# Ecogenomics/CheckM

Measured on NVIDIA H100. Metric: genomes/hour, higher is better.
Workload: dtype int16 (SSV) / u8 (MSV) / int16 (Viterbi) / f32 (Forward, domain definition)

## Files before the change

checkm_b200/csrc/kernels_vitp.cu:

```cuda
#include "engine.hpp"
#include "device_utils.cuh"
#include "stages.hpp"

namespace ckm {

constexpr uint32_t VP_FLOORW = 0xD800D800u;
constexpr int      VP_FLOOR  = -10240;
constexpr uint32_t VP_TFLOORW = 0xC000C000u;

__device__ __forceinline__ int vp_lo(uint32_t w) { return (int)(int16_t)(w & 0xffffu); }
__device__ __forceinline__ int vp_hi(uint32_t w) { return (int)w >> 16; }

__device__ __forceinline__ void vit_pass(const FilterParams &p, const Candidate &cd) {
  const int pos = atomicAdd(p.out_count, 1);
  if (pos < p.out_cap) p.out[pos] = cd;
  if (p.dense_passed != nullptr) atomicOr_u8(p.dense_passed, (int64_t)p.model_slot[cd.model] * p.nseq + cd.seq, 4);
}
__device__ __forceinline__ void vit_redo(const FilterParams &p, const Candidate &cd) {
  const int pos = atomicAdd(p.redo_count, 1);
  if (pos < p.redo_cap) p.redo[pos] = cd;
}
__device__ __forceinline__ int vitp_class(int vq) { return vq == 0 ? -1 : (vq <= 8 ? vq / 2 - 1 : vq / 4 + 1); }

__global__ void vit_count_kernel(FilterParams p, int32_t *cnt) {
  const int n = min(*p.in_count, p.in_cap);
  for (int i = blockIdx.x * blockDim.x + threadIdx.x; i < n; i += gridDim.x * blockDim.x) {
    const Candidate cd = p.in[i];
    if (!(cd.P > p.F2)) vit_pass(p, cd);
    else if (p.ms[cd.model].vq == 0) vit_redo(p, cd);
    else atomicAdd(cnt + cd.model, 1);
  }
}

__global__ void __launch_bounds__(1024) vit_scan_kernel(FilterParams p, int32_t nmodels, const int32_t *cnt, int32_t *off, int32_t *choff) {
  __shared__ int ws[2][32];
  const int lane = threadIdx.x & 31, warp = threadIdx.x >> 5;
  int run_pairs = 0, run_chunks = 0;
  for (int c = 0; c < N_BLK_CLASSES; ++c) {
    if (threadIdx.x == 0) p.vit_cls_chunks[c] = run_chunks;
    for (int b = 0; b < nmodels; b += 1024) {
      const int m = b + threadIdx.x;
      const int v = (m < nmodels && vitp_class(p.ms[m].vq) == c) ? cnt[m] : 0, h = (v + VITP_CHUNK - 1) / VITP_CHUNK;
      int sv = v, sh = h;
#pragma unroll
      for (int o = 1; o < 32; o <<= 1) {
        const int a = __shfl_up_sync(0xffffffffu, sv, o), d = __shfl_up_sync(0xffffffffu, sh, o);
        if (lane >= o) { sv += a; sh += d; }
      }
      if (lane == 31) { ws[0][warp] = sv; ws[1][warp] = sh; }
      __syncthreads();
      if (warp == 0) {
        int tv = ws[0][lane], th = ws[1][lane];
#pragma unroll
        for (int o = 1; o < 32; o <<= 1) {
          const int a = __shfl_up_sync(0xffffffffu, tv, o), d = __shfl_up_sync(0xffffffffu, th, o);
          if (lane >= o) { tv += a; th += d; }
        }
        ws[0][lane] = tv; ws[1][lane] = th;
      }
      __syncthreads();
      if (v > 0) {
        off[m] = run_pairs + (warp ? ws[0][warp - 1] : 0) + sv - v;
        choff[m] = run_chunks + (warp ? ws[1][warp - 1] : 0) + sh - h;
      }
      run_pairs += ws[0][31]; run_chunks += ws[1][31];
      __syncthreads();
    }
  }
  if (threadIdx.x == 0) p.vit_cls_chunks[N_BLK_CLASSES] = run_chunks;
}

__global__ void vit_scatter_kernel(FilterParams p, const int32_t *cnt, int32_t *fill, const int32_t *off, const int32_t *choff) {
  const int n = min(*p.in_count, p.in_cap);
  for (int i = blockIdx.x * blockDim.x + threadIdx.x; i < n; i += gridDim.x * blockDim.x) {
    const int m = p.in[i].model;
    if (!(p.in[i].P > p.F2) || p.ms[m].vq == 0) continue;
    const int r = atomicAdd(fill + m, 1), pos = off[m] + r;
    p.vit_idx[pos] = i;
    if (r % VITP_CHUNK == 0) p.vit_chunks[choff[m] + r / VITP_CHUNK] = make_int2(pos, off[m] + min(r + VITP_CHUNK, cnt[m]));
  }
}

int launch_vit_group(const FilterParams &p, int32_t nmodels, int32_t *ws, int grid, cudaStream_t st) {
  int32_t *cnt = ws, *fill = ws + nmodels, *off = ws + 2 * (size_t)nmodels, *choff = ws + 3 * (size_t)nmodels;
  cudaError_t e = cudaMemsetAsync(ws, 0, sizeof(int32_t) * 2 * (size_t)nmodels, st);
  if (e != cudaSuccess) return cuda_fail(e, "cudaMemsetAsync(vit groups)");
  vit_count_kernel<<<grid, 256, 0, st>>>(p, cnt);
  vit_scan_kernel<<<1, 1024, 0, st>>>(p, nmodels, cnt, off, choff);
  vit_scatter_kernel<<<grid, 256, 0, st>>>(p, cnt, fill, off, choff);
  e = cudaGetLastError();
  return e == cudaSuccess ? CKM_OK : cuda_fail(e, "vit grouping launch");
}

constexpr int VITP_THREADS = 128;

__host__ __device__ constexpr int vitp_smem_bytes(int W, bool tsmem) { return KPAD * W * 32 * 4 + (tsmem ? W * 64 * 16 : 0); }
__host__ __device__ constexpr int vitp_min_blocks(int W) { return W <= 4 ? 4 : (W <= 10 ? 3 : 2); }

template <int W, bool TSMEM>
__global__ void __launch_bounds__(VITP_THREADS, vitp_min_blocks(W)) vitp_kernel(FilterParams p, int cls) {
  extern __shared__ __align__(16) uint4 vsm[];
  __shared__ int s_chunk, s_next;
  __shared__ ModelScalars s_ms;
  uint32_t *esm = reinterpret_cast<uint32_t *>(vsm);
  uint4 *tws = vsm + KPAD * W * 8;
  const int lane = threadIdx.x & 31;
  const uint32_t sel = (lane == 0) ? 0x1054u : 0x3210u;
  const int c0 = p.vit_cls_chunks[cls], nch = p.vit_cls_chunks[cls + 1] - c0;
  for (;;) {
    __syncthreads();
    if (threadIdx.x == 0) {
      const int k = atomicAdd(p.vit_work + cls, 1);
      s_chunk = k;
      if (k < nch) {
        s_next = p.vit_chunks[c0 + k].x;
        s_ms = p.ms[p.in[p.vit_idx[s_next]].model];
      }
    }
    __syncthreads();
    const int k = s_chunk;
    if (k >= nch) break;
    const int2 ch = p.vit_chunks[c0 + k];
    const ModelScalars &ms = s_ms;
    {
      const uint4 *esrc = reinterpret_cast<const uint4 *>(p.rwp + ms.blk_off * 32 * (KPAD / 2));
      for (int z = threadIdx.x; z < KPAD * W * 8; z += VITP_THREADS) vsm[z] = __ldg(esrc + z);
      if (TSMEM) {
        const uint4 *tsrc = p.twp + ms.blk_off * 32;
        for (int z = threadIdx.x; z < W * 64; z += VITP_THREADS) tws[(z & 1) * (W * 32) + (z >> 1)] = __ldg(tsrc + z);
      }
    }
    uint4 tr0[TSMEM ? 1 : W], tr1[TSMEM ? 1 : W];
    if (!TSMEM) {
      const uint4 *tsrc = p.twp + ms.blk_off * 32;
#pragma unroll
      for (int w = 0; w < W; ++w) { tr0[TSMEM ? 0 : w] = __ldg(tsrc + (w * 32 + lane) * 2); tr1[TSMEM ? 0 : w] = __ldg(tsrc + (w * 32 + lane) * 2 + 1); }
    }
#define TR0(w) (TSMEM ? tws[(w) * 32 + lane] : tr0[TSMEM ? 0 : (w)])
#define TR1(w) (TSMEM ? tws[W * 32 + (w) * 32 + lane] : tr1[TSMEM ? 0 : (w)])
    __syncthreads();
    const uint32_t *erow = esm + lane;
    const int ddbound = ms.ddbound_w, cap = 32767 - (int)ms.vit_emax;
    const int e_move = ms.xw_e_move, e_loop = ms.xw_e_loop;
    for (;;) {
      int j = 0;
      if (lane == 0) j = atomicAdd(&s_next, 1);
      j = __shfl_sync(0xffffffffu, j, 0);
      if (j >= ch.y) break;
      const Candidate *cin = p.in + p.vit_idx[j];
      const int s = cin->seq, L = p.len[s];
      bool redo = false;
      const int tmove = p.tmove_w[s];
      const int cost = -tmove - (int)ms.vit_tbm + 64;
      const bool c1 = (cost - (int)ms.xw_e_loop <= 22528) && (cost <= 22240);
      const bool c1p = (cost - (int)ms.xw_e_loop <= 16384);
      redo = !c1;
      float vsc = 0.0f;
      if (!redo) {
        uint32_t Mx[W], Ix[W], Dx[W];
#pragma unroll
        for (int w = 0; w < W; ++w) { Mx[w] = VP_FLOORW; Ix[w] = VP_FLOORW; Dx[w] = VP_FLOORW; }
        int xN = ms.base_w, xB = xN + tmove, xJ = -32768, xC = -32768;
        const uint32_t *rp = reinterpret_cast<const uint32_t *>(p.res + p.off[s]);
        const int nw = (L + 3) >> 2;
        uint32_t wcur = (nw > 0) ? __ldg(rp) : 0u;
        bool stop = false;
        for (int q = 0; q < nw && !stop; ++q) {
          const uint32_t wnext = (q + 1 < nw) ? __ldg(rp + q + 1) : 0u;
#pragma unroll
          for (int rr = 0; rr < 4; ++rr) {
            if (q * 4 + rr >= L) { stop = true; break; }
            const uint32_t *ew = erow + ((wcur >> (8 * rr)) & 0xffu) * (W * 32);
            const uint32_t shM = __shfl_sync(0xffffffffu, Mx[W - 1], (lane + 31) & 31);
            const uint32_t shI = __shfl_sync(0xffffffffu, Ix[W - 1], (lane + 31) & 31);
            const uint32_t shD = __shfl_sync(0xffffffffu, Dx[W - 1], (lane + 31) & 31);
            const uint32_t pm0 = __byte_perm(shM, VP_FLOORW, sel), pi0 = __byte_perm(shI, VP_FLOORW, sel), pd0 = __byte_perm(shD, VP_FLOORW, sel);
            const uint32_t xBw = __byte_perm((uint32_t)xB, 0u, 0x1010u);
            uint32_t md[W];
            uint32_t xEw = VP_FLOORW, dmw = VP_FLOORW;
#pragma unroll
            for (int w = W - 1; w >= 0; --w) {
              const uint32_t pm = (w > 0) ? Mx[w - 1] : pm0, pi = (w > 0) ? Ix[w - 1] : pi0, pd = (w > 0) ? Dx[w - 1] : pd0;
              const uint4 t0 = TR0(w), t1 = TR1(w);
              uint32_t sv = __viaddmax_s16x2(xBw, t0.x, VP_FLOORW);
              sv = __viaddmax_s16x2(pm, t0.y, sv);
              sv = __viaddmax_s16x2(pi, t0.z, sv);
              sv = __viaddmax_s16x2(pd, t0.w, sv);
              sv = __viaddmax_s16x2(sv, ew[w * 32], VP_FLOORW);
              const uint32_t nI = __viaddmax_s16x2(Ix[w], t1.z, __viaddmax_s16x2(Mx[w], t1.y, VP_FLOORW));
              md[w] = __viaddmax_s16x2(sv, t1.x, VP_FLOORW);
              Mx[w] = sv; Ix[w] = nI;
            }
#pragma unroll
            for (int w = 0; w + 1 < W; w += 2) { xEw = __vimax3_s16x2(xEw, Mx[w], Mx[w + 1]); dmw = __vimax3_s16x2(dmw, md[w], md[w + 1]); }
            if (W & 1) { xEw = __vimax3_s16x2(xEw, Mx[W - 1], Mx[W - 1]); dmw = __vimax3_s16x2(dmw, md[W - 1], md[W - 1]); }
            const int xE = __reduce_max_sync(0xffffffffu, max(vp_lo(xEw), vp_hi(xEw)));
            if (xE >= cap) { redo = true; stop = true; break; }
            xC = max(xC, xE + e_move);
            xJ = max(xJ, xE + e_loop);
            xB = max(xJ + tmove, xN + tmove);
            const int Dmax = __reduce_max_sync(0xffffffffu, max(vp_lo(dmw), vp_hi(dmw)));
            if (Dmax + ddbound > xB) {
              if (!c1p) { redo = true; stop = true; break; }
              uint32_t Bb = VP_FLOORW, Tb = 0u;
#pragma unroll
              for (int w = 0; w < W; ++w) { const uint32_t tdd = TR1(w).w; Bb = __viaddmax_s16x2(Bb, tdd, md[w]); Tb = __viaddmax_s16x2(Tb, __vimax3_s16x2(tdd, VP_TFLOORW, VP_TFLOORW), VP_TFLOORW); }
              uint32_t Bs = Bb, Ts = Tb;
#pragma unroll
              for (int o = 1; o < 32; o <<= 1) {
                const uint32_t Bl = __shfl_up_sync(0xffffffffu, Bs, o), Tl = __shfl_up_sync(0xffffffffu, Ts, o);
                if (lane >= o) { Bs = __viaddmax_s16x2(Bl, Ts, Bs); Ts = __viaddmax_s16x2(Ts, Tl, VP_TFLOORW); }
              }
              uint32_t din = __shfl_up_sync(0xffffffffu, Bs, 1), Tex = __shfl_up_sync(0xffffffffu, Ts, 1);
              if (lane == 0) { din = VP_FLOORW; Tex = 0u; }
              const uint32_t lowexit = __shfl_sync(0xffffffffu, Bs, 31);
              const uint32_t dmid = __byte_perm(lowexit, VP_FLOORW, 0x1054u);
              din = __viaddmax_s16x2(dmid, Tex, din);
              uint32_t d = din;
#pragma unroll
              for (int w = 0; w < W; ++w) { Dx[w] = d; d = __viaddmax_s16x2(d, TR1(w).w, md[w]); }
            } else {
              const uint32_t shd = __shfl_sync(0xffffffffu, md[W - 1], (lane + 31) & 31);
#pragma unroll
              for (int w = W - 1; w >= 1; --w) Dx[w] = md[w - 1];
              Dx[0] = __byte_perm(shd, VP_FLOORW, sel);
            }
          }
          wcur = wnext;
        }
        if (!redo && xC <= VP_FLOOR + e_move) redo = true;
        if (!redo) {
          vsc = __fsub_rn(__fadd_rn((float)xC, (float)tmove), (float)ms.base_w);
          vsc = __fdiv_rn(vsc, ms.scale_w);
          vsc = __fsub_rn(vsc, 3.0f);
        }
      }
      Candidate cd = *cin;
      if (redo) {
        if (lane == 0) vit_redo(p, cd);
        continue;
      }
      cd.vitsc = vsc;
      const float seq_score = __fdiv_rn(__fsub_rn(vsc, cd.filtersc), 0.69314718055994529f);
      const double P = gumbel_surv((double)seq_score, (double)ms.evparam[2], (double)ms.evparam[3]);
      cd.P = P;
      if (lane == 0) {
        if (p.dense_vit != nullptr) p.dense_vit[(int64_t)p.model_slot[cd.model] * p.nseq + s] = vsc;
        if (P <= p.F2) vit_pass(p, cd);
      }
    }
#undef TR0
#undef TR1
  }
}

template <int W, bool TSMEM>
static int launch_vitp_w(const FilterParams &p, int cls, int grid, cudaStream_t st) {
  constexpr int sm = vitp_smem_bytes(W, TSMEM);
  if (sm > 48 * 1024) {
    cudaError_t e = cudaFuncSetAttribute(vitp_kernel<W, TSMEM>, cudaFuncAttributeMaxDynamicSharedMemorySize, sm);
    if (e != cudaSuccess) return cuda_fail(e, "cudaFuncSetAttribute(vitp)");
  }
  vitp_kernel<W, TSMEM><<<grid, VITP_THREADS, sm, st>>>(p, cls);
  cudaError_t e = cudaGetLastError();
  return e == cudaSuccess ? CKM_OK : cuda_fail(e, "vitp_kernel launch");
}

__global__ void all_pairs_kernel(Candidate *out, int32_t *count, const int32_t *slot_model, int32_t nslots, int32_t nseq) {
  const int64_t n = (int64_t)nslots * nseq;
  for (int64_t i = blockIdx.x * (int64_t)blockDim.x + threadIdx.x; i < n; i += (int64_t)gridDim.x * blockDim.x) {
    Candidate cd;
    cd.seq = (int32_t)(i % nseq); cd.model = slot_model[i / nseq]; cd.usc = 0.0f; cd.filtersc = 0.0f; cd.vitsc = 0.0f; cd.fwdsc = 0.0f; cd.P = 1.0;
    out[i] = cd;
  }
  if (blockIdx.x == 0 && threadIdx.x == 0) *count = (int32_t)n;
}
int launch_all_pairs(Candidate *out, int32_t *count, const int32_t *slot_model, int32_t nslots, int32_t nseq, cudaStream_t st) {
  all_pairs_kernel<<<592, 256, 0, st>>>(out, count, slot_model, nslots, nseq);
  cudaError_t e = cudaGetLastError();
  return e == cudaSuccess ? CKM_OK : cuda_fail(e, "all_pairs_kernel launch");
}

int launch_vitp(const FilterParams &p, int cls, int grid, cudaStream_t st) {
  switch (cls) {
    case 0: return launch_vitp_w<1, false>(p, cls, grid, st);
    case 1: return launch_vitp_w<2, false>(p, cls, grid, st);
    case 2: return launch_vitp_w<3, false>(p, cls, grid, st);
    case 3: return launch_vitp_w<4, false>(p, cls, grid, st);
    case 4: return launch_vitp_w<6, true>(p, cls, grid, st);
    case 5: return launch_vitp_w<8, true>(p, cls, grid, st);
    case 6: return launch_vitp_w<10, true>(p, cls, grid, st);
    case 7: return launch_vitp_w<12, true>(p, cls, grid, st);
    case 8: return launch_vitp_w<14, true>(p, cls, grid, st);
    case 9: return launch_vitp_w<16, true>(p, cls, grid, st);
  }
  set_error("launch_vitp: bad class"); return CKM_EINVAL;
}

}
```

Measured before the change: 35780.

## Add half-warp Viterbi kernel for the two smallest model classes

Adds a half_vitp_kernel in which each 16-lane half-warp processes its own sequence, with each lane holding twice as many stripe registers. The two smallest model-width classes (W=1,2) now use it instead of the full-warp kernel. The aim is to double sequences per warp for short models, where full-warp shuffles and reductions underuse the lanes. The cost is more registers per thread, 16-wide shuffles and some divergence when the two halves finish at different times.

```diff
diff --git a/checkm_b200/csrc/kernels_vitp.cu b/checkm_b200/csrc/kernels_vitp.cu
--- a/checkm_b200/csrc/kernels_vitp.cu
+++ b/checkm_b200/csrc/kernels_vitp.cu
@@ -254,16 +254,197 @@
   }
 }
 
+template <int W>
+__global__ void __launch_bounds__(VITP_THREADS, vitp_min_blocks(W)) half_vitp_kernel(FilterParams p, int cls) {
+  constexpr int HW = 2 * W;
+  constexpr unsigned FULL = 0xffffffffu;
+  extern __shared__ __align__(16) uint4 vsm[];
+  __shared__ int s_chunk, s_next;
+  __shared__ ModelScalars s_ms;
+  const uint32_t *esm = reinterpret_cast<const uint32_t *>(vsm);
+  const int lane = threadIdx.x & 31, hl = lane & 15;
+  const unsigned hmask = 0xffffu << (lane & 16);
+  const int src = (hl + 15) & 15;
+  const uint32_t sel = (hl == 0) ? 0x1054u : 0x3210u;
+  const int c0 = p.vit_cls_chunks[cls], nch = p.vit_cls_chunks[cls + 1] - c0;
+  for (;;) {
+    __syncthreads();
+    if (threadIdx.x == 0) {
+      const int k = atomicAdd(p.vit_work + cls, 1);
+      s_chunk = k;
+      if (k < nch) {
+        s_next = p.vit_chunks[c0 + k].x;
+        s_ms = p.ms[p.in[p.vit_idx[s_next]].model];
+      }
+    }
+    __syncthreads();
+    const int k = s_chunk;
+    if (k >= nch) break;
+    const int2 ch = p.vit_chunks[c0 + k];
+    const ModelScalars &ms = s_ms;
+    {
+      const uint4 *esrc = reinterpret_cast<const uint4 *>(p.rwp + ms.blk_off * 32 * (KPAD / 2));
+      for (int z = threadIdx.x; z < KPAD * W * 8; z += VITP_THREADS) vsm[z] = __ldg(esrc + z);
+    }
+    uint4 tr0[HW], tr1[HW];
+    {
+      const uint4 *tsrc = p.twp + ms.blk_off * 32;
+#pragma unroll
+      for (int w = 0; w < HW; ++w) {
+        const int t = (w % W) * 32 + 2 * hl + w / W;
+        tr0[w] = __ldg(tsrc + t * 2); tr1[w] = __ldg(tsrc + t * 2 + 1);
+      }
+    }
+    __syncthreads();
+    const uint32_t *erow = esm + 2 * hl;
+    const int ddbound = ms.ddbound_w, cap = 32767 - (int)ms.vit_emax;
+    const int e_move = ms.xw_e_move, e_loop = ms.xw_e_loop;
+    int j = 0, L = 0, nw = 0, q = 0, tmove = 0, xN = 0, xB = 0, xJ = 0, xC = 0;
+    bool need = true, active = true, c1p = false, redo = false, stop = false;
+    const uint32_t *rp = nullptr;
+    uint32_t wcur = 0u;
+    uint32_t Mx[HW], Ix[HW], Dx[HW];
+#pragma unroll
+    for (int w = 0; w < HW; ++w) { Mx[w] = VP_FLOORW; Ix[w] = VP_FLOORW; Dx[w] = VP_FLOORW; }
+    for (;;) {
+      while (need) {
+        int jj = 0;
+        if (hl == 0) jj = atomicAdd(&s_next, 1);
+        jj = __shfl_sync(hmask, jj, 0, 16);
+        if (jj >= ch.y) { active = false; need = false; L = 0; nw = 0; q = 0; wcur = 0u; stop = false; break; }
+        const Candidate *cin = p.in + p.vit_idx[jj];
+        const int s = cin->seq;
+        tmove = p.tmove_w[s];
+        const int cost = -tmove - (int)ms.vit_tbm + 64;
+        if (!((cost - (int)ms.xw_e_loop <= 22528) && (cost <= 22240))) {
+          if (hl == 0) vit_redo(p, *cin);
+          continue;
+        }
+        c1p = (cost - (int)ms.xw_e_loop <= 16384);
+        j = jj; L = p.len[s]; nw = (L + 3) >> 2; q = 0;
+        rp = reinterpret_cast<const uint32_t *>(p.res + p.off[s]);
+        wcur = (nw > 0) ? __ldg(rp) : 0u;
+        xN = ms.base_w; xB = xN + tmove; xJ = -32768; xC = -32768;
+        redo = false; stop = false; need = false;
+#pragma unroll
+        for (int w = 0; w < HW; ++w) { Mx[w] = VP_FLOORW; Ix[w] = VP_FLOORW; Dx[w] = VP_FLOORW; }
+      }
+      if (!__any_sync(FULL, active)) break;
+      bool fin = false;
+      for (;;) {
+        const uint32_t wnext = (q + 1 < nw) ? __ldg(rp + q + 1) : 0u;
+        const int rem = L - q * 4;
+#pragma unroll
+        for (int rr = 0; rr < 4; ++rr) {
+          const bool live = rr < rem && !stop;
+          const uint32_t *ew = erow + ((wcur >> (8 * rr)) & 0xffu) * (W * 32);
+          const uint32_t shM = __shfl_sync(FULL, Mx[HW - 1], src, 16);
+          const uint32_t shI = __shfl_sync(FULL, Ix[HW - 1], src, 16);
+          const uint32_t shD = __shfl_sync(FULL, Dx[HW - 1], src, 16);
+          const uint32_t pm0 = __byte_perm(shM, VP_FLOORW, sel), pi0 = __byte_perm(shI, VP_FLOORW, sel), pd0 = __byte_perm(shD, VP_FLOORW, sel);
+          const uint32_t xBw = __byte_perm((uint32_t)xB, 0u, 0x1010u);
+          uint32_t md[HW];
+          uint32_t xEw = VP_FLOORW, dmw = VP_FLOORW;
+#pragma unroll
+          for (int w = HW - 1; w >= 0; --w) {
+            const uint32_t pm = (w > 0) ? Mx[w - 1] : pm0, pi = (w > 0) ? Ix[w - 1] : pi0, pd = (w > 0) ? Dx[w - 1] : pd0;
+            const uint4 t0 = tr0[w], t1 = tr1[w];
+            uint32_t sv = __viaddmax_s16x2(xBw, t0.x, VP_FLOORW);
+            sv = __viaddmax_s16x2(pm, t0.y, sv);
+            sv = __viaddmax_s16x2(pi, t0.z, sv);
+            sv = __viaddmax_s16x2(pd, t0.w, sv);
+            sv = __viaddmax_s16x2(sv, ew[(w % W) * 32 + w / W], VP_FLOORW);
+            const uint32_t nI = __viaddmax_s16x2(Ix[w], t1.z, __viaddmax_s16x2(Mx[w], t1.y, VP_FLOORW));
+            md[w] = __viaddmax_s16x2(sv, t1.x, VP_FLOORW);
+            Mx[w] = sv; Ix[w] = nI;
+          }
+#pragma unroll
+          for (int w = 0; w < HW; w += 2) { xEw = __vimax3_s16x2(xEw, Mx[w], Mx[w + 1]); dmw = __vimax3_s16x2(dmw, md[w], md[w + 1]); }
+          uint32_t red = __vmaxs2(__byte_perm(xEw, dmw, 0x5410u), __byte_perm(xEw, dmw, 0x7632u));
+#pragma unroll
+          for (int o = 8; o >= 1; o >>= 1) red = __vmaxs2(red, __shfl_xor_sync(FULL, red, o));
+          const int xE = vp_lo(red), Dmax = vp_hi(red);
+          if (live) {
+            if (xE >= cap) { redo = true; stop = true; }
+            else {
+              xC = max(xC, xE + e_move);
+              xJ = max(xJ, xE + e_loop);
+              xB = max(xJ + tmove, xN + tmove);
+            }
+          }
+          const uint32_t shd = __shfl_sync(FULL, md[HW - 1], src, 16);
+          if (live && !stop && Dmax + ddbound > xB) {
+            if (!c1p) { redo = true; stop = true; }
+            else {
+              uint32_t Bb = VP_FLOORW, Tb = 0u;
+#pragma unroll
+              for (int w = 0; w < HW; ++w) { const uint32_t tdd = tr1[w].w; Bb = __viaddmax_s16x2(Bb, tdd, md[w]); Tb = __viaddmax_s16x2(Tb, __vimax3_s16x2(tdd, VP_TFLOORW, VP_TFLOORW), VP_TFLOORW); }
+              uint32_t Bs = Bb, Ts = Tb;
+#pragma unroll
+              for (int o = 1; o < 16; o <<= 1) {
+                const uint32_t Bl = __shfl_up_sync(hmask, Bs, o, 16), Tl = __shfl_up_sync(hmask, Ts, o, 16);
+                if (hl >= o) { Bs = __viaddmax_s16x2(Bl, Ts, Bs); Ts = __viaddmax_s16x2(Ts, Tl, VP_TFLOORW); }
+              }
+              uint32_t din = __shfl_up_sync(hmask, Bs, 1, 16), Tex = __shfl_up_sync(hmask, Ts, 1, 16);
+              if (hl == 0) { din = VP_FLOORW; Tex = 0u; }
+              const uint32_t lowexit = __shfl_sync(hmask, Bs, 15, 16);
+              const uint32_t dmid = __byte_perm(lowexit, VP_FLOORW, 0x1054u);
+              din = __viaddmax_s16x2(dmid, Tex, din);
+              uint32_t d = din;
+#pragma unroll
+              for (int w = 0; w < HW; ++w) { Dx[w] = d; d = __viaddmax_s16x2(d, tr1[w].w, md[w]); }
+            }
+          } else {
+#pragma unroll
+            for (int w = HW - 1; w >= 1; --w) Dx[w] = md[w - 1];
+            Dx[0] = __byte_perm(shd, VP_FLOORW, sel);
+          }
+        }
+        wcur = wnext;
+        ++q;
+        fin = active && (stop || q >= nw);
+        if (__any_sync(FULL, fin)) break;
+      }
+      if (fin) {
+        if (!redo && xC <= VP_FLOOR + e_move) redo = true;
+        if (hl == 0) {
+          Candidate cd = p.in[p.vit_idx[j]];
+          if (redo) vit_redo(p, cd);
+          else {
+            float vsc = __fsub_rn(__fadd_rn((float)xC, (float)tmove), (float)ms.base_w);
+            vsc = __fdiv_rn(vsc, ms.scale_w);
+            vsc = __fsub_rn(vsc, 3.0f);
+            cd.vitsc = vsc;
+            const float seq_score = __fdiv_rn(__fsub_rn(vsc, cd.filtersc), 0.69314718055994529f);
+            const double P = gumbel_surv((double)seq_score, (double)ms.evparam[2], (double)ms.evparam[3]);
+            cd.P = P;
+            if (p.dense_vit != nullptr) p.dense_vit[(int64_t)p.model_slot[cd.model] * p.nseq + cd.seq] = vsc;
+            if (P <= p.F2) vit_pass(p, cd);
+          }
+        }
+        need = true;
+      }
+    }
+  }
+}
+
+template <class Kernel>
+static int launch_vitp_k(Kernel kern, int sm, const FilterParams &p, int cls, int grid, cudaStream_t st) {
+  if (sm > 48 * 1024) {
+    cudaError_t e = cudaFuncSetAttribute(kern, cudaFuncAttributeMaxDynamicSharedMemorySize, sm);
+    if (e != cudaSuccess) return cuda_fail(e, "cudaFuncSetAttribute(vitp)");
+  }
+  kern<<<grid, VITP_THREADS, sm, st>>>(p, cls);
+  cudaError_t e = cudaGetLastError();
+  return e == cudaSuccess ? CKM_OK : cuda_fail(e, "vitp_kernel launch");
+}
 template <int W, bool TSMEM>
 static int launch_vitp_w(const FilterParams &p, int cls, int grid, cudaStream_t st) {
-  constexpr int sm = vitp_smem_bytes(W, TSMEM);
-  if (sm > 48 * 1024) {
-    cudaError_t e = cudaFuncSetAttribute(vitp_kernel<W, TSMEM>, cudaFuncAttributeMaxDynamicSharedMemorySize, sm);
-    if (e != cudaSuccess) return cuda_fail(e, "cudaFuncSetAttribute(vitp)");
-  }
-  vitp_kernel<W, TSMEM><<<grid, VITP_THREADS, sm, st>>>(p, cls);
-  cudaError_t e = cudaGetLastError();
-  return e == cudaSuccess ? CKM_OK : cuda_fail(e, "vitp_kernel launch");
+  return launch_vitp_k(vitp_kernel<W, TSMEM>, vitp_smem_bytes(W, TSMEM), p, cls, grid, st);
+}
+template <int W>
+static int launch_vitp_half(const FilterParams &p, int cls, int grid, cudaStream_t st) {
+  return launch_vitp_k(half_vitp_kernel<W>, vitp_smem_bytes(W, false), p, cls, grid, st);
 }
 
 __global__ void all_pairs_kernel(Candidate *out, int32_t *count, const int32_t *slot_model, int32_t nslots, int32_t nseq) {
@@ -283,8 +464,8 @@
 
 int launch_vitp(const FilterParams &p, int cls, int grid, cudaStream_t st) {
   switch (cls) {
-    case 0: return launch_vitp_w<1, false>(p, cls, grid, st);
-    case 1: return launch_vitp_w<2, false>(p, cls, grid, st);
+    case 0: return launch_vitp_half<1>(p, cls, grid, st);
+    case 1: return launch_vitp_half<2>(p, cls, grid, st);
     case 2: return launch_vitp_w<3, false>(p, cls, grid, st);
     case 3: return launch_vitp_w<4, false>(p, cls, grid, st);
     case 4: return launch_vitp_w<6, true>(p, cls, grid, st);
```

New measurement: 35970, median of 6. Within noise of the previous version (+0.5%).
